# justinhj/minbpe-cc

Hardware: AMD Instinct MI355X
Metric: bpe_train_merges_per_sec (higher is better)
Workload: dtype u16; 1 GPU; BASELINE config 4: SplitMix64(seed 42) uniform-random bytes, 4294967296 bytes whole job, basic encoder (one chunk), vocab 32000, lexicographic tie-break; a step is ONE WHOLE TRAINING (pair-count scan, stream and table setup, every merge up to the vocabulary: 31744 merges); corpus_bytes=4294967296, vocab_size=32000

## Files before the change

### include/mbpe.h

```cpp
#ifndef MBPE_H
#define MBPE_H

#include <stdint.h>

#ifdef __cplusplus
extern "C" {
#endif

#define MBPE_API __attribute__((visibility("default")))

#define MBPE_MAX_VOCAB_BASIC   65534u
#define MBPE_MAX_VOCAB_ENDBIT  32766u
#define MBPE_MAX_VOCAB_CHUNKED 65518u
#define MBPE_MAX_VOCAB_WIDE    16777216u
#define MBPE_NO_BARRIER 0xFFFFFFFFu

typedef enum {
    MBPE_NEED_EXCHANGE =  1,
    MBPE_OK            =  0,
    MBPE_ERR_ARG       = -1,
    MBPE_ERR_NO_DEVICE = -2,
    MBPE_ERR_HIP       = -3,
    MBPE_ERR_VOCAB     = -4,
    MBPE_ERR_STATE     = -5,
// ... 76 lines not shown
MBPE_API int mbpe_train_sequences(mbpe_ctx *ctx, uint32_t n_sequences, uint32_t *merges_done_out);

MBPE_API int mbpe_train_result(mbpe_ctx *ctx, uint32_t *merges_out, int32_t *counts_out,
                               uint32_t cap_merges, uint32_t *n_merges_out);

MBPE_API int mbpe_train_lexical(mbpe_ctx *ctx, const uint8_t *text, uint64_t n_bytes,
                                const uint64_t *chunk_off, uint64_t n_chunks,
                                uint32_t vocab_size,
                                uint32_t *merges_out, int32_t *counts_out,
                                uint32_t *n_merges_out, mbpe_stats *stats_out);

MBPE_API int mbpe_train(mbpe_ctx *ctx, const uint8_t *text, uint64_t n_bytes,
                        const uint64_t *chunk_off, uint64_t n_chunks, uint32_t vocab_size,
                        int conflict_resolution,
                        uint32_t *merges_out, int32_t *counts_out,
                        uint32_t *n_merges_out, mbpe_stats *stats_out);

MBPE_API int mbpe_get_stats(mbpe_ctx *ctx, mbpe_stats *out);


MBPE_API int mbpe_get_stream(mbpe_ctx *ctx, uint32_t *tokens_out, uint8_t *chunk_end_out,
                             uint64_t cap, uint64_t *n_out);

MBPE_API int mbpe_stream_device(mbpe_ctx *ctx, const void **slots_out, uint64_t *n_slots_out,
                                uint32_t *slot_bits_out, uint32_t *end_bit_out, uint32_t *barrier_out);

MBPE_API int mbpe_table_device(mbpe_ctx *ctx, const void **cells_out, uint32_t *vshift_out);

MBPE_API int mbpe_get_pairs(mbpe_ctx *ctx, uint32_t *first_out, uint32_t *second_out,
                            int32_t *count_out, uint64_t cap, uint64_t *n_out);

MBPE_API int mbpe_compact(mbpe_ctx *ctx);

MBPE_API int mbpe_set_option(mbpe_ctx *ctx, const char *name, int64_t value);


MBPE_API int mbpe_encode_chunks(int device_id, const uint8_t *text, uint64_t n_bytes,
                                const uint64_t *chunk_off, uint64_t n_chunks,
                                const uint32_t *merges, uint32_t n_merges,
                                uint32_t *tokens_out, uint64_t cap, uint64_t *n_out,
                                uint32_t *n_passes_out);

MBPE_API int mbpe_encode_chunks_device(int device_id, const uint8_t *text, uint64_t n_bytes,
                                       const uint64_t *chunk_off, uint64_t n_chunks,
                                       const uint32_t *merges, uint32_t n_merges,
                                       uint32_t *tokens_dev_out, uint64_t cap, uint64_t *n_out,
                                       uint32_t *n_passes_out);

typedef struct mbpe_encoder mbpe_encoder;
MBPE_API int  mbpe_encoder_create(int device_id, const uint32_t *merges, uint32_t n_merges, mbpe_encoder **out);
MBPE_API void mbpe_encoder_destroy(mbpe_encoder *e);

MBPE_API int  mbpe_encoder_encode(mbpe_encoder *e, const uint8_t *text, uint64_t n_bytes, int text_on_device,
                                  const uint64_t *chunk_off, uint64_t n_chunks,
                                  void *tokens_out, uint64_t cap, uint32_t token_bits, int out_on_device,
                                  uint64_t *chunk_tok_off_out, uint64_t *n_out, uint32_t *n_passes_out);

MBPE_API int  mbpe_encoder_set_option(mbpe_encoder *e, const char *name, int64_t value);

MBPE_API int  mbpe_encoder_kernel_ms(const mbpe_encoder *e, float *ms_out);

MBPE_API int  mbpe_encoder_pass_tokens(const mbpe_encoder *e, uint64_t *tokens_out, uint32_t cap, uint32_t *n_out);

MBPE_API int  mbpe_encoder_alloc_count(const mbpe_encoder *e, uint64_t *n_out);


// ... 48 lines not shown
```

### minbpe-cc_amd/csrc/kernels.hip

```cpp
#include "mbpe_dev.h"
#include <hip/hip_ext.h>

#include <cstdlib>

namespace mbpe {

namespace {

constexpr int kWave = 64;
constexpr uint32_t kSent = 0x10000u;

__device__ __forceinline__ uint32_t lane_id() { return threadIdx.x & (kWave - 1); }
__device__ __forceinline__ uint32_t rfl(uint32_t v) { return __builtin_amdgcn_readfirstlane(v); }

typedef unsigned int u32x4 __attribute__((ext_vector_type(4)));

__device__ __forceinline__ uint32_t wave_from_next(uint32_t v, uint32_t edge) {
    return (uint32_t)__builtin_amdgcn_update_dpp((int)edge, (int)v, 0x130, 0xf, 0xf, false);
}
__device__ __forceinline__ uint32_t wave_from_prev(uint32_t v, uint32_t edge) {
    return (uint32_t)__builtin_amdgcn_update_dpp((int)edge, (int)v, 0x138, 0xf, 0xf, false);
}

#define MBPE_GLOBAL_AS __attribute__((address_space(1)))
// ... 583 lines not shown
            }
            const uint32_t issued = pc_generic_range(hist, bp, text, n, n_full, r_begin, v_end);
            __syncthreads();
            const PcCheck ck = pc_check(hist, issued, red);
            if (ck.sum != resid + ck.issued) {
#pragma unroll
                for (int k = 0; k < kPcWords / 4 / kPcThreads; ++k)
                    reinterpret_cast<uint4 *>(hist)[k * kPcThreads + threadIdx.x] =
                        resid ? my_snap[k * kPcThreads + threadIdx.x] : make_uint4(0, 0, 0, 0);
                __syncthreads();
                pc_slow_range(hist, bp, text, n, n_full, r_begin, v_end);
            }
        }
    }
    __syncthreads();
    PC_STAMP();
    pc_flush(hist, bp);
    const bool ends_here = n_full == 0 ? blockIdx.x == 0 : (v_begin < n_full && v_end == n_full);
    if (ends_here && threadIdx.x == 0) {
        uint64_t i = n_full * 16;
        if (i > 0 && !straddle_counted) --i;
        if (n_full * 16 == n) i = n;
        for (; i + 1 < n; ++i) atomicAdd(&bp[((uint32_t)text[i] << 8) | text[i + 1]], 1u);
    }
#ifdef MBPE_PC_STAMPS
    __builtin_amdgcn_s_waitcnt(0);
    __syncthreads();
    PC_STAMP();
    if (threadIdx.x == 0) for (; n_stamp < 16; ++n_stamp) stamps[n_stamp] = 0;
#endif
}


template <bool MASKED>
__global__ void k_widen(const uint8_t *__restrict__ text, uint64_t n, const uint8_t *__restrict__ endmask,
                        uint16_t *__restrict__ tok, uint64_t n_padded) {
    uint64_t vec = (uint64_t)blockIdx.x * blockDim.x + threadIdx.x;
    const uint64_t stride = (uint64_t)gridDim.x * blockDim.x;
    const uint64_t n_vec = n_padded / 16;
    for (; vec < n_vec; vec += stride) {
        const uint64_t byte0 = vec * 16;
        uint32_t w[4] = {0, 0, 0, 0};
        uint32_t ends = 0;
        if (byte0 + 16 <= n) {
            uint4 q = *reinterpret_cast<const uint4 *>(text + byte0);
            w[0] = q.x; w[1] = q.y; w[2] = q.z; w[3] = q.w;
        } else {
            for (uint64_t i = byte0; i < n; ++i)
                w[(i - byte0) >> 2] |= (uint32_t)text[i] << (8 * ((i - byte0) & 3));
        }
        if (MASKED && byte0 < n) ends = reinterpret_cast<const uint16_t *>(endmask)[vec];
        uint32_t o[8];
#pragma unroll
        for (int i = 0; i < 16; i += 2) {
            uint32_t t0 = (w[i >> 2] >> (8 * (i & 3))) & 0xFFu;
            uint32_t t1 = (w[(i + 1) >> 2] >> (8 * ((i + 1) & 3))) & 0xFFu;
            if (MASKED) {
                t0 |= ((ends >> i) & 1u) << 15;
                t1 |= ((ends >> (i + 1)) & 1u) << 15;
            }
            if (byte0 + i >= n) t0 = kHole;
            if (byte0 + i + 1 >= n) t1 = kHole;
            o[i >> 1] = t0 | (t1 << 16);
        }
        uint4 *dst = reinterpret_cast<uint4 *>(tok + byte0);
        dst[0] = make_uint4(o[0], o[1], o[2], o[3]);
        dst[1] = make_uint4(o[4], o[5], o[6], o[7]);
    }
}

__global__ void k_widen_barrier(const uint8_t *__restrict__ text, uint64_t n, const uint8_t *__restrict__ endmask,
                                uint16_t *__restrict__ tok, uint64_t n_slots) {
    uint64_t vec = (uint64_t)blockIdx.x * blockDim.x + threadIdx.x;
    const uint64_t stride = (uint64_t)gridDim.x * blockDim.x;
    const uint64_t n_vec = n_slots / 16;
    for (; vec < n_vec; vec += stride) {
        const uint64_t byte0 = vec * 8;
        uint32_t w[2] = {0, 0};
        uint32_t ends = 0;
        if (byte0 + 8 <= n) {
            const uint2 q = *reinterpret_cast<const uint2 *>(text + byte0);
            w[0] = q.x; w[1] = q.y;
        } else {
            for (uint64_t i = byte0; i < n; ++i) w[(i - byte0) >> 2] |= (uint32_t)text[i] << (8 * ((i - byte0) & 3));
        }
        if (byte0 < n) ends = endmask[vec];
        uint32_t o[8];
#pragma unroll
        for (int i = 0; i < 8; ++i) {
            uint32_t t = (w[i >> 2] >> (8 * (i & 3))) & 0xFFu;
            uint32_t e = ((ends >> i) & 1u) ? kBarrier : kHole;
            if (byte0 + i >= n) { t = kHole; e = kHole; }
            o[i] = t | (e << 16);
        }
        uint4 *dst = reinterpret_cast<uint4 *>(tok + vec * 16);
        dst[0] = make_uint4(o[0], o[1], o[2], o[3]);
        dst[1] = make_uint4(o[4], o[5], o[6], o[7]);
    }
}


template <int MODE>
// ... 225 lines not shown
    if (t == 0xFFFFFFFFu) return;
    const uint32_t nb = blockIdx.x, per = (nb + kRunThreads - 1) / kRunThreads;
    RunSeg acc = run_none();
    for (uint32_t i = threadIdx.x * per; i < nb && i < (threadIdx.x + 1) * per; ++i) acc = run_join(acc, run_unpack(part[i]));
    pre[threadIdx.x] = run_pack(acc);
    const uint64_t base = (uint64_t)blockIdx.x * kRunChunk;
    run_chunk_join(sin, n_tiles, base, segs, sh);
    if (threadIdx.x == 0) {
        RunSeg run = run_none();
        for (int i = 0; i < kRunThreads; ++i) run = run_join(run, run_unpack(pre[i]));
        for (int i = 0; i < kRunThreads; ++i) {
            const RunSeg mine = run_unpack(sh[i]);
            sh[i] = run_pack(run);
            run = run_join(run, mine);
        }
    }
    __syncthreads();
    RunSeg run = run_unpack(sh[threadIdx.x]);
    const unsigned long long edge = le ? ((unsigned long long)le->tail_run_hi << 32) | le->tail_run_lo : 0ull;
    const uint32_t edge_tok = le ? le->tail0 : kHole;
    for (int i = 0; i < kRunPerThread; ++i) {
        const uint32_t k = threadIdx.x * kRunPerThread + i;
        const bool reach = le && edge_tok != kHole && (run.empty || (run.full && run.token == edge_tok));
        const unsigned long long rb = run.len + (reach ? edge : 0ull);
        const RunSeg here = run_unpack(segs[k]);
        segs[k] = (rb & 1ull) | (rb >= 2 ? 2ull : 0ull);
        run = run_join(run, here);
    }
    __syncthreads();
    for (uint32_t i = threadIdx.x; i < kRunChunk; i += kRunThreads)
        if (base + i < n_tiles) run_in[base + i] = (uint32_t)segs[i];
}

__global__ __launch_bounds__(kMergeThreads) void k_summarize(const uint16_t *__restrict__ tok,
                                                             TileSum *__restrict__ sums, uint32_t n_tiles) {
    const uint32_t waves_per_block = kMergeThreads / kWave;
    const uint32_t n_waves = gridDim.x * waves_per_block;
    for (uint32_t tile = blockIdx.x * waves_per_block + threadIdx.x / kWave; tile < n_tiles; tile += n_waves) {
        const uint4 q = reinterpret_cast<const uint4 *>(tok)[(uint64_t)tile * kWave + lane_id()];
        uint32_t s[8];
        unpack8(q, s);
        uint4 sum;
        bool live = true;
#pragma unroll
        for (int j = 0; j < 8; ++j) live = live && s[j] != kHole;
        if (__ballot(!live) == 0ull) {
            const uint32_t lane = lane_id();
            const uint32_t t0 = rlane(s[7], kWave - 1);
            uint32_t last_diff = 0;
#pragma unroll
            for (int j = 0; j < 8; ++j) last_diff = s[j] != t0 ? (uint32_t)j + 1u : last_diff;
            const unsigned long long dm = __ballot(last_diff != 0u);
            uint32_t run = kTile;
            if (dm) {
                const uint32_t hl = 63u - (uint32_t)__builtin_clzll(dm);
                run = kTile - (hl * 8u + rlane(last_diff, hl));
            }
            sum = sum_to_u4(rlane(s[0], 0), rlane(s[1], 0), rlane(s[6], kWave - 1), t0, kTile, run);
            (void)lane;
        } else {
            sum = wave_summary(s);
        }
        if (lane_id() == 0) reinterpret_cast<uint4 *>(sums)[tile] = sum;
    }
}


constexpr int kArgmaxThreads = 256;

__global__ __launch_bounds__(kArgmaxThreads) void k_argmax(PairTable t, const DevCtl *ctl,
                                                           unsigned long long *best) {
    __shared__ unsigned long long wbest[kArgmaxThreads / kWave];
    const uint32_t n = table_size(t, ctl);
    unsigned long long b = 0;
    for (uint32_t i = blockIdx.x * blockDim.x + threadIdx.x; i < n; i += gridDim.x * blockDim.x) {
        const unsigned long long p = entry_packed(t, i);
        b = p > b ? p : b;
    }
    b = wave_max_u64(b);
    if (lane_id() == 0) wbest[threadIdx.x / kWave] = b;
    __syncthreads();
    if (threadIdx.x == 0) {
#pragma unroll
        for (int k = 1; k < kArgmaxThreads / kWave; ++k) b = wbest[k] > b ? wbest[k] : b;
        if (b) atomicMax(best, b);
    }
}

constexpr int kHierThreads = 256;
constexpr int kHierItems = kBlockSize / kHierThreads;

struct Top2 { unsigned long long v1, v2; uint32_t i1; };

__device__ __forceinline__ Top2 top2_merge(Top2 a, unsigned long long bv1, unsigned long long bv2, uint32_t bi1) {
    Top2 r;
    if (bv1 > a.v1) { r.v1 = bv1; r.i1 = bi1; r.v2 = a.v1 > bv2 ? a.v1 : bv2; }
// ... 1737 lines not shown
                }
            }
            outq = fused_tile_pf<MODE, DIAG, true, TT>(t0.q, s, h, old_x, old_y, old_z, lut, X0, tile, sout, hdr_adj, LR, dc,
                                                       dc_on, wave_rm, wrote_sum, lr_rsrc, adj_pitch, stage, chg, renamed, &ti,
                                                       need_rename, t_rsrc, use_t);
            if (TT && need_rename) {
                tt_rename<MODE>(s, h, ti, run_in[tile]);
                outq = fused_tile_pf<MODE, DIAG, true, TT>(t0.q, s, h, old_x, old_y, old_z, lut, X0, tile, sout, hdr_adj, LR,
                                                           dc, dc_on, wave_rm, wrote_sum, lr_rsrc, adj_pitch, stage, chg, true,
                                                           &ti, need_rename, t_rsrc, use_t);
            }
        }
        if (!wrote_sum && lane == 0) reinterpret_cast<uint4 *>(sout)[tile] = make_uint4(old_x, old_y, old_z, 0u);
        MBPE_GLOBAL_AS char *obase =
            (MBPE_GLOBAL_AS char *)uniform_ptr(reinterpret_cast<uintptr_t>(dst) + (uint64_t)tile * (kWave * 16u));
        u32x4 oq; oq.x = outq.x; oq.y = outq.y; oq.z = outq.z; oq.w = outq.w;
        __builtin_nontemporal_store(oq, (MBPE_GLOBAL_AS u32x4 *)(obase + lane * 16u));

        if (!v1) break;
        tile += n_waves;
#pragma unroll
        for (int d = 0; d + 1 < kDepth; ++d) ring[d] = ring[d + 1];
        ring[kDepth - 1] = t_new;
    }
    }
    if (dc_on) dc_flush(dc, LR);
    if (lane == 0 && wave_rm) atomicAdd(&ctl->rm, wave_rm);
    if (TT) {
        tt_flush(ti, hdr_m);
    }
}

__global__ __launch_bounds__(256) void k_pair_cells_fold(uint32_t *__restrict__ T, uint32_t *__restrict__ LR, const DevCtl *ctl) {
    __shared__ uint32_t rows[256];
    const uint32_t n = ctl->batch_n;
    if (n < ctl->cells_min || !ctl->cells_on) return;
    const uint32_t pitch = lr_pitch(256u + ctl->k_done);
    uint32_t hits = 0;
    const uint32_t t = threadIdx.x;
    for (uint32_t j = blockIdx.x; j < n; j += gridDim.x) {
        uint32_t *tj = T + (size_t)j * 65536u;
        rows[t] = 0;
        __syncthreads();
        uint32_t col = 0;
#pragma unroll 8
        for (uint32_t x = 0; x < 256u; ++x) {
            const uint32_t v = tj[x * 256u + t];
            if (__ballot(v != 0u) == 0ull) continue;
            if (v) tj[x * 256u + t] = 0;
            col += v;
            const uint32_t rs = wave_sum(v);
            if (lane_id() == 0 && rs) atomicAdd(&rows[x], rs);
        }
        __syncthreads();
        if (col) LR[lr_idx(pitch, t, j, 1u)] += col;
        if (rows[t]) LR[lr_idx(pitch, t, j, 0u)] += rows[t];
        hits += col;
        __syncthreads();
    }
    hits = wave_sum(hits);
    if (lane_id() == 0 && hits) atomicAdd(const_cast<uint32_t *>(&ctl->cell_hits), hits);
}


__global__ __launch_bounds__(kWave) void k_adj_sums(const uint32_t *__restrict__ hdr_adj, BatchState *bs, const DevCtl *ctl) {
    const uint32_t n = ctl->batch_n;
    if (n < 2) return;
    for (uint32_t j = blockIdx.x; j < n; j += gridDim.x) {
        uint32_t in = 0, out = 0;
        for (uint32_t p = threadIdx.x; p < n; p += kWave) { in += hdr_adj[p * ctl->adj_pitch + j]; out += hdr_adj[j * ctl->adj_pitch + p]; }
        in = wave_sum(in);
        out = wave_sum(out);
        if (threadIdx.x == 0) { bs->adj_in[j] = in; bs->adj_out[j] = out; }
    }
}

constexpr uint32_t kLrChunk = 4096;
__global__ __launch_bounds__(256) void k_delta_max(const uint32_t *__restrict__ LR, BatchState *bs, const DevCtl *ctl) {
    const uint32_t n_keys = ctl->batch_n;
    if (n_keys < 2) return;
    const uint32_t X = 256u + ctl->k_done;
    const uint32_t pitch = lr_pitch(X);
    const uint32_t chunks = (X + kLrChunk - 1u) / kLrChunk;
    const uint32_t n_items = 2u * n_keys * chunks;
    for (uint32_t item = blockIdx.x; item < n_items; item += gridDim.x) {
        const uint32_t row = item / chunks, x0 = (item - row * chunks) * kLrChunk;
        const uint32_t j = row >> 1, side = row & 1u, Xj = X + j;
// ... 771 lines not shown
        else if ((endbit) == kBarrier) { constexpr int M = 2; __VA_ARGS__; }               \
        else { constexpr int M = 0; __VA_ARGS__; }                                         \
    } while (0)

void launch_fill_u32(hipStream_t s, uint32_t *p, uint64_t n, uint32_t v) {
    if (!n) return;
    hipLaunchKernelGGL(k_fill_u32, dim3(blocks_for(n, 256, 4096)), dim3(256), 0, s, p, n, v);
}

void launch_fill_u16(hipStream_t s, uint16_t *p, uint64_t n, uint16_t v) {
    if (!n) return;
    hipLaunchKernelGGL(k_fill_u16, dim3(blocks_for(n, 256, 4096)), dim3(256), 0, s, p, n, v);
}

size_t pair_count_scratch_bytes(int n_workgroups) {
    const size_t wgs = (size_t)(n_workgroups < 1 ? 1 : n_workgroups);
    return wgs * kPcWords * 4 + wgs * 16 * 8;
}

void launch_pair_count_u8(hipStream_t s, const uint8_t *text, uint64_t n, const uint8_t *endmask,
                          uint32_t *bp, int n_workgroups, uint32_t *scratch, hipEvent_t start, hipEvent_t stop) {
    if (n < 2) return;
    uint64_t n_vec = n / 16;
    uint64_t max_wg = (n_vec + kPcThreads * kPcVpl - 1) / (kPcThreads * kPcVpl);
    if ((uint64_t)n_workgroups > max_wg) n_workgroups = (int)max_wg;
    if (n_workgroups < 1) n_workgroups = 1;
    if (endmask)
        hipExtLaunchKernelGGL(k_pair_count_u8<true>, dim3(n_workgroups), dim3(kPcThreads), 0, s, start, stop, 0, text, n, endmask, bp, scratch);
    else
        hipExtLaunchKernelGGL(k_pair_count_u8_fast, dim3(n_workgroups), dim3(kPcThreads), 0, s, start, stop, 0, text, n, bp, scratch);
}

void launch_widen(hipStream_t s, const uint8_t *text, uint64_t n, const uint8_t *endmask, uint16_t *tok,
                  uint64_t n_slots_padded) {
    if (!n_slots_padded) return;
    int blocks = blocks_for(n_slots_padded / 16, 256, 8192);
    if (endmask)
        hipLaunchKernelGGL(k_widen<true>, dim3(blocks), dim3(256), 0, s, text, n, endmask, tok, n_slots_padded);
    else
        hipLaunchKernelGGL(k_widen<false>, dim3(blocks), dim3(256), 0, s, text, n, endmask, tok, n_slots_padded);
}

void launch_widen_barrier(hipStream_t s, const uint8_t *text, uint64_t n, const uint8_t *endmask, uint16_t *tok,
                          uint64_t n_slots) {
    if (!n_slots) return;
    hipLaunchKernelGGL(k_widen_barrier, dim3(blocks_for(n_slots / 16, 256, 8192)), dim3(256), 0, s, text, n, endmask, tok,
                       n_slots);
}

void launch_summarize(hipStream_t s, const uint16_t *tok, TileSum *sums, uint32_t n_tiles, int n_cus) {
    if (!n_tiles) return;
    hipLaunchKernelGGL(k_summarize, dim3(tile_grid(n_tiles, n_cus)), dim3(kMergeThreads), 0, s, tok, sums, n_tiles);
}

void launch_table_init(hipStream_t s, const uint32_t *bp, PairTable t, DevCtl *ctl) {
    hipLaunchKernelGGL(k_table_init, dim3(65536 / 256), dim3(256), 0, s, bp, t, ctl);
}

void launch_table_rehash(hipStream_t s, PairTable t, DevCtl *ctl) {
    hipLaunchKernelGGL(k_table_rehash, dim3((t.ecap + 255) / 256), dim3(256), 0, s, t, ctl);
}

void launch_argmax(hipStream_t s, PairTable t, const DevCtl *ctl, unsigned long long *best, bool hierarchical) {
    if (hierarchical) {
        hipLaunchKernelGGL(k_argmax_hier, dim3(1), dim3(kHierThreads), 0, s, t, ctl, best);
        return;
    }
    int blocks = blocks_for(t.ecap, kArgmaxThreads * 4, 1024);
    hipLaunchKernelGGL(k_argmax, dim3(blocks), dim3(kArgmaxThreads), 0, s, t, ctl, best);
}

size_t first_state_bytes() { return sizeof(FirstState); }

// ... 292 lines not shown
```

### minbpe-cc_amd/csrc/mbpe_dev.h

```cpp
#ifndef MBPE_DEV_H
#define MBPE_DEV_H

#include <hip/hip_runtime.h>
#include <stdint.h>

namespace mbpe {

constexpr uint32_t kHole = 0xFFFFu;
constexpr uint32_t kEndBit = 0x8000u;
constexpr uint32_t kBarrier = 0xFFEEu;

constexpr int kTile = 512;
constexpr int kMergeThreads = 256;
#ifndef MBPE_LUT_THREADS
#define MBPE_LUT_THREADS 1024
#endif
constexpr int kLutThreads = MBPE_LUT_THREADS;
constexpr int kSlotsPerLane = 8;

struct __attribute__((aligned(16))) TileSum {
    uint16_t head0, head1;
    uint16_t tail1, tail0;
    uint16_t n_live;
    uint16_t tail_run;
// ... 121 lines not shown
    uint32_t skip_pos[kSkipMax];
    unsigned long long skip_packed[kSkipMax];
};

inline uint32_t batch_header_words(uint32_t adj_pitch) { return (uint32_t)kBatchMax + adj_pitch * adj_pitch; }
__host__ __device__ inline uint32_t lr_pitch(uint32_t ids) { return (ids + 63u) & ~63u; }
__host__ __device__ inline unsigned long long lr_words(uint32_t ids, uint32_t n_pairs) {
    return 2ull * (n_pairs ? n_pairs : 1u) * lr_pitch(ids);
}

constexpr uint32_t kErrTableFull   = 1u;
constexpr uint32_t kErrNegCount    = 2u;
constexpr uint32_t kErrMissingPair = 4u;
constexpr uint32_t kErrCountRange  = 8u;
constexpr uint32_t kErrHotSkipped  = 16u;

__host__ __device__ inline unsigned long long pack_best(int32_t count, uint32_t key) {
    return ((unsigned long long)(uint32_t)count << 32) | (uint32_t)(~key);
}

struct Launch {
    hipStream_t stream;
};

void launch_fill_u32(hipStream_t s, uint32_t *p, uint64_t n, uint32_t v);
void launch_fill_u16(hipStream_t s, uint16_t *p, uint64_t n, uint16_t v);

size_t pair_count_scratch_bytes(int n_workgroups);
void launch_pair_count_u8(hipStream_t s, const uint8_t *text, uint64_t n,
                          const uint8_t *endmask, uint32_t *bp, int n_workgroups, uint32_t *scratch,
                          hipEvent_t start = nullptr, hipEvent_t stop = nullptr);

void launch_widen(hipStream_t s, const uint8_t *text, uint64_t n, const uint8_t *endmask,
                  uint16_t *tok, uint64_t n_slots_padded);
void launch_widen_barrier(hipStream_t s, const uint8_t *text, uint64_t n, const uint8_t *endmask,
                          uint16_t *tok, uint64_t n_slots);

void launch_summarize(hipStream_t s, const uint16_t *tok, TileSum *sums, uint32_t n_tiles, int n_cus);

void launch_table_init(hipStream_t s, const uint32_t *bp, PairTable t, DevCtl *ctl);
void launch_table_rehash(hipStream_t s, PairTable t, DevCtl *ctl);

void launch_argmax(hipStream_t s, PairTable t, const DevCtl *ctl, unsigned long long *best, bool hierarchical);

size_t first_state_bytes();
void launch_first_init(hipStream_t s, void *fs);
void launch_first_tiebreak(hipStream_t s, PairTable t, const DevCtl *ctl, unsigned long long *best, void *fs,
                           const uint16_t *tok, const uint16_t *tok_other, const TileSum *sums, uint32_t n_tiles,
                           uint32_t endbit, int n_cus, int seq,
                           int phase = 0 ,
                           const RankEdge *right_edge = nullptr, uint32_t *xf = nullptr ,
                           int rank = 0, int n_ranks = 1);

void launch_merge(hipStream_t s, uint16_t *tok, uint16_t *tok_other, const TileSum *sums, TileSum *side,
                  uint32_t n_tiles, uint32_t *chg, const unsigned long long *best, uint32_t new_id,
                  uint32_t endbit, uint32_t *LR, DevCtl *ctl, uint32_t *m_adj ,
                  const RankEdge *left_edge, const RankEdge *right_edge, int n_cus, int seq,
                  unsigned long long *run_part ,
                  uint32_t *run_in ,
                  const BatchState *bs ,
                  int hot_possible = 1 ,
                  int only = -1 );
void launch_run_lengths(hipStream_t s, const TileSum *sums, uint32_t n_tiles, const unsigned long long *best, const DevCtl *ctl,
                        int seq, const BatchState *bs, unsigned long long *run_part, const RankEdge *left_edge, uint32_t *run_in);

void launch_apply(hipStream_t s, PairTable t, DevCtl *ctl, const unsigned long long *best,
                  uint32_t new_id, uint32_t *LR, const uint32_t *gm_gadj,
// ... 50 lines not shown
```

### minbpe-cc_amd/csrc/train.cpp

```cpp
#include "mbpe.h"
#include "mbpe_dev.h"
#include "wide.h"
#include "hip_host.h"

#include <dlfcn.h>
#include <rccl/rccl.h>

#include <algorithm>
#include <chrono>
#include <cstddef>
#include <cstdio>
#include <cstring>
#include <map>
#include <string>
#include <unordered_map>
#include <vector>

using namespace mbpe;

namespace {

#define HIPCHK(expr) MBPE_HIP_CHECK(expr, false)

uint64_t round_up(uint64_t v, uint64_t m) { return (v + m - 1) / m * m; }
// ... 776 lines not shown
        init.first_mode = c->opt_first ? 1u : 0u;
        init.adj_pitch = c->adj_pitch;
        init.cells_on = c->pair_cells ? 1u : 0u;
        init.cells_min = c->opt_pair_cells > 0 ? 2u : kCellsMinBatch;
        c->h_ctl = init;
        HIPCHK(hipMemcpyAsync(c->ctl, &c->h_ctl, sizeof(DevCtl), hipMemcpyHostToDevice, c->stream));
    }
    HIPCHK(hipMemsetAsync(c->best, 0, ((size_t)c->n_target + 2) * 8, c->stream));

    uint64_t want = 65536 + 2 * batch_headroom(c, (uint32_t)c->opt_batch);
    want = std::max<uint64_t>(want, n / 8);
    want = std::min<uint64_t>(want, table_cap_limit(c));
    int rc = use_dense(c) ? alloc_table_dense(c) : alloc_table(c, (uint32_t)want);
    if (rc != MBPE_OK) return rc;

    rc = ensure_pc_scratch(c);
    if (rc != MBPE_OK) return rc;
    pool_trim(c);
    HIPCHK(hipEventRecord(c->ev0, c->stream));
    if (n >= 2) launch_pair_count_u8(c->stream, c->d_text, n, c->d_endmask, c->xb0, c->n_cus, c->pc_scratch);
    c->cur = 0;
    if (c->barrier) {
        launch_widen_barrier(c->stream, c->d_text, n, c->d_endmask, c->tok[0], c->n_slots);
        launch_summarize(c->stream, c->tok[0], c->sums, c->n_tiles, c->n_cus);
        const double ms_compact = c->stats.ms_compact;
        rc = do_compact(c);
        if (rc != MBPE_OK) return rc;
        c->stats.n_compactions--;
        c->stats.ms_compact = ms_compact;
        tfree(c, c->tok[0]);
        pool_trim(c);
        HIPCHK(tmalloc(c, &c->tok[0], c->cap_slots * 2));
    } else {
        launch_widen(c->stream, c->d_text, n, c->d_endmask, c->tok[0], c->n_slots);
        launch_summarize(c->stream, c->tok[0], c->sums, c->n_tiles, c->n_cus);
    }
    if (is_multi(c)) {
        uint32_t *hdr = c->xb0 + 65536;
        launch_rank_edge(c->stream, c->sums, c->n_tiles, reinterpret_cast<RankEdge *>(hdr + 2) + c->rank, c->ctl, hdr);
        const uint64_t p = pairs_scanned(c);
        for (uint32_t i = 0; i < kPairCountWords; ++i) c->h_pcount[i] = (uint32_t)(p >> (16 * i)) & 0xFFFFu;
        HIPCHK(hipMemcpyAsync(hdr + c->hdr_words, c->h_pcount, sizeof(c->h_pcount), hipMemcpyHostToDevice, c->stream));
    }
    return MBPE_OK;
}

static void update_hot_possible(mbpe_ctx *c, unsigned long long top_count, uint64_t merges) {
    c->last_top = top_count;
    if (c->comm_external) { c->hot_possible = 1; return; }
    const unsigned long long live = c->h_ctl.n_live;
    const unsigned long long eaten = merges * top_count;
    c->hot_possible = !(live > eaten && top_count * 8192ull < (live - eaten) * (unsigned long long)std::max(1, c->n_ranks));
}

static inline bool first_sharded(const mbpe_ctx *c) { return c->opt_first && is_multi(c); }

static void begin_finish_a(mbpe_ctx *c) {
    const uint32_t endbit = endbit_of(c);
    if (is_multi(c)) {
        uint32_t *hdr = c->xb0 + 65536;
        launch_boundary_pairs(c->stream, c->xb0, hdr, c->n_ranks, endbit, hdr + c->hdr_words);
        launch_compose_edges(c->stream, hdr, c->rank, c->n_ranks, c->d_left, c->d_right);
        launch_pair_total(c->stream, c->xb0, hdr + c->hdr_words, 0, nullptr, c->ctl);
    } else {
        launch_pair_total(c->stream, c->xb0, nullptr, pairs_scanned(c), nullptr, c->ctl);
    }
    launch_table_init(c->stream, c->xb0, c->tab, c->ctl);
    launch_argmax(c->stream, c->tab, c->ctl, c->best, use_hier(c));
// ... 1024 lines not shown
            HIPCHK(hipMemcpy(rowbuf.data(), c->tab.cells + (size_t)tr * tpr * 1024, rowbuf.size() * 4,
                             hipMemcpyDeviceToHost));
            for (uint32_t fr = 0; fr < 32; ++fr)
                for (uint32_t tc = 0; tc < used_tiles; ++tc)
                    for (uint32_t sc = 0; sc < 32; ++sc) {
                        const uint32_t v = rowbuf[(size_t)tc * 1024 + fr * 32 + sc];
                        if (v & kPresent) recs.push_back({tr * 32 + fr, tc * 32 + sc, (int32_t)(v & ~kPresent)});
                    }
        }
        uint64_t o = recs.size();
        if (o > n) { mbpe_host::set_last_error("pair table holds more pairs than counted"); return MBPE_ERR_OVERFLOW; }
        for (uint64_t i = 0; i < o; ++i) {
            first_out[i] = recs[i].f;
            second_out[i] = recs[i].s;
            if (count_out) count_out[i] = recs[i].c;
        }
        if (o != n) { mbpe_host::set_last_error("pair table holds fewer pairs than counted"); return MBPE_ERR_OVERFLOW; }
        return MBPE_OK;
    }
    std::vector<uint32_t> keys(n);
    std::vector<int32_t> cnts(n);
    if (n) {
        HIPCHK(hipMemcpy(keys.data(), c->tab.ekey, n * 4, hipMemcpyDeviceToHost));
        HIPCHK(hipMemcpy(cnts.data(), c->tab.ecnt, n * 4, hipMemcpyDeviceToHost));
    }
    for (uint64_t i = 0; i < n; ++i) {
        first_out[i] = keys[i] >> 16;
        second_out[i] = keys[i] & 0xFFFFu;
        if (count_out) count_out[i] = cnts[i];
    }
    return MBPE_OK;
}

int mbpe_compact(mbpe_ctx *c) {
    if (!c) return MBPE_ERR_ARG;
    if (!c->begun) { mbpe_host::set_last_error("mbpe_compact before mbpe_train_begin"); return MBPE_ERR_STATE; }
    HIPCHK(hipSetDevice(c->device));
    if (c->wide_active) return MBPE_OK;
    int rc = sync_ctl(c);
    if (rc != MBPE_OK) return rc;
    return do_compact(c);
}


static int comm_allreduce(mbpe_ctx *c, uint32_t *buf, size_t count) {
    Rccl &r = rccl();
    if (!r.ok || !c->nccl_comm) { mbpe_host::set_last_error("RCCL communicator not initialised"); return MBPE_ERR_COMM; }
    int rc = r.AllReduce(buf, buf, count, (int)ncclUint32, (int)ncclSum, c->nccl_comm, c->stream);
    if (rc != 0) {
        mbpe_host::set_last_error(std::string("ncclAllReduce: ") + r.GetErrorString(rc));
        return MBPE_ERR_COMM;
    }
    return MBPE_OK;
}

int mbpe_comm_unique_id(uint8_t *id_out) {
    if (!id_out) return MBPE_ERR_ARG;
    Rccl &r = rccl();
    if (!r.ok) { mbpe_host::set_last_error(r.why); return MBPE_ERR_COMM; }
    static_assert(sizeof(ncclUniqueId) == MBPE_COMM_ID_BYTES, "unique id size");
    ncclUniqueId id;
    int rc = r.GetUniqueId(&id);
    if (rc != 0) { mbpe_host::set_last_error(std::string("ncclGetUniqueId: ") + r.GetErrorString(rc)); return MBPE_ERR_COMM; }
    memcpy(id_out, &id, sizeof(id));
    return MBPE_OK;
}
// ... 39 lines not shown
```

### minbpe-cc_amd/python/mbpe/__init__.py

```python
import ctypes
import os

import numpy as np

_PKG_DIR = os.path.dirname(os.path.dirname(os.path.dirname(os.path.abspath(__file__))))
LIB_PATH = os.environ.get("MBPE_LIB") or os.path.join(_PKG_DIR, "libmbpe.so")

OK = 0
NEED_EXCHANGE = 1
ERR_ARG, ERR_NO_DEVICE, ERR_HIP, ERR_VOCAB, ERR_STATE = -1, -2, -3, -4, -5
ERR_OOM, ERR_REGEX, ERR_SPLIT_GAP, ERR_COMM, ERR_OVERFLOW, ERR_IO = -6, -7, -8, -9, -10, -11
COMM_ID_BYTES = 128

EXPORTS = [
    "mbpe_last_error", "mbpe_version", "mbpe_create", "mbpe_destroy", "mbpe_load_corpus",
    "mbpe_pair_count_u8", "mbpe_train_begin", "mbpe_train_steps", "mbpe_train_sequences", "mbpe_train_result",
    "mbpe_train_lexical", "mbpe_train", "mbpe_get_stats", "mbpe_get_stream", "mbpe_stream_device", "mbpe_table_device", "mbpe_get_pairs", "mbpe_compact",
    "mbpe_set_option", "mbpe_comm_unique_id", "mbpe_comm_init", "mbpe_comm_init_external",
    "mbpe_comm_exchange_buffer", "mbpe_comm_exchange_done", "mbpe_presplit",
    "mbpe_split_count", "mbpe_split_offsets", "mbpe_split_has_gaps", "mbpe_split_starts", "mbpe_split_ends",
    "mbpe_split_free", "mbpe_load_corpus_ranges", "mbpe_split_pattern", "mbpe_encode_chunks",
    "mbpe_encode_chunks_device", "mbpe_decoder_create", "mbpe_decoder_destroy", "mbpe_decode_tokens",
    "mbpe_decode_slots", "mbpe_decoder_kernel_ms", "mbpe_decode_stream", "mbpe_encoder_create",
    "mbpe_encoder_destroy", "mbpe_encoder_encode", "mbpe_encoder_set_option", "mbpe_encoder_kernel_ms",
    "mbpe_encoder_alloc_count", "mbpe_encoder_pass_tokens",
]
TOK_EXPORTS = [
    "mbpe_tok_create", "mbpe_tok_destroy", "mbpe_tok_set_special_tokens", "mbpe_tok_train", "mbpe_tok_set_merges",
    "mbpe_tok_get_merges", "mbpe_tok_save", "mbpe_tok_load", "mbpe_tok_encode", "mbpe_tok_encode_device",
    "mbpe_tok_decode", "mbpe_tok_decode_device", "mbpe_tok_encode_batch_device",
]


class Stats(ctypes.Structure):
    _fields_ = [
        ("n_bytes", ctypes.c_uint64), ("n_chunks", ctypes.c_uint64), ("n_slots", ctypes.c_uint64),
        ("n_live", ctypes.c_uint64), ("n_merges", ctypes.c_uint32), ("n_compactions", ctypes.c_uint32),
        ("n_pairs", ctypes.c_uint64), ("ms_pair_count", ctypes.c_float), ("ms_begin", ctypes.c_float),
        ("ms_steps", ctypes.c_float), ("pair_count_launches", ctypes.c_uint32), ("merge_launches", ctypes.c_uint32),
        ("ms_merge_kernel", ctypes.c_float), ("n_batches", ctypes.c_uint32),
        ("n_fused", ctypes.c_uint32), ("n_fused_dropped", ctypes.c_uint32), ("cut_conflict", ctypes.c_uint32),
        ("cut_bucket", ctypes.c_uint32), ("cut_single", ctypes.c_uint32), ("cut_full", ctypes.c_uint32),
        ("n_validation_drops", ctypes.c_uint32), ("ms_grow_table", ctypes.c_float), ("ms_compact", ctypes.c_float),
        ("n_table_grows", ctypes.c_uint32), ("n_sel_fallback", ctypes.c_uint32),
        ("fused_launches", ctypes.c_uint32), ("ms_fused_kernel", ctypes.c_float), ("fused_slots", ctypes.c_uint64),
        ("n_sel_retry", ctypes.c_uint32), ("adapt_limit", ctypes.c_uint32), ("n_sel_blocks", ctypes.c_uint64), ("size_hist", ctypes.c_uint32 * 8),
        ("n_skipped", ctypes.c_uint32), ("n_skip_cut", ctypes.c_uint32),
        ("exchange_words", ctypes.c_uint64), ("exchanges", ctypes.c_uint32), ("pad_", ctypes.c_uint32),
        ("fused_live_tokens", ctypes.c_uint64), ("ms_pair_count_kernel", ctypes.c_float), ("pad2_", ctypes.c_uint32),
    ]
# ... 12 lines not shown


_lib = None


def lib():
    global _lib
    if _lib is not None:
        return _lib
    if not os.path.exists(LIB_PATH):
        raise ImportError("libmbpe.so is not built (%s); run __graft_entry__.build()" % LIB_PATH)
    L = ctypes.CDLL(LIB_PATH)
    vp, u64, u32, i32, i64 = ctypes.c_void_p, ctypes.c_uint64, ctypes.c_uint32, ctypes.c_int, ctypes.c_int64
    L.mbpe_last_error.restype = ctypes.c_char_p
    L.mbpe_version.restype = ctypes.c_char_p
    L.mbpe_create.argtypes = [i32, ctypes.POINTER(vp)]
    L.mbpe_destroy.argtypes = [vp]
    L.mbpe_destroy.restype = None
    L.mbpe_load_corpus.argtypes = [vp, vp, u64, vp, u64, i32]
    L.mbpe_pair_count_u8.argtypes = [vp, vp]
    L.mbpe_train_begin.argtypes = [vp, u32]
    L.mbpe_train_steps.argtypes = [vp, u32, vp]
    L.mbpe_train_sequences.argtypes = [vp, u32, vp]
    L.mbpe_train_result.argtypes = [vp, vp, vp, u32, vp]
    L.mbpe_train_lexical.argtypes = [vp, vp, u64, vp, u64, u32, vp, vp, vp, vp]
    L.mbpe_train.argtypes = [vp, vp, u64, vp, u64, u32, i32, vp, vp, vp, vp]
    L.mbpe_get_stats.argtypes = [vp, vp]
    L.mbpe_get_stream.argtypes = [vp, vp, vp, u64, vp]
    L.mbpe_stream_device.argtypes = [vp, ctypes.POINTER(vp), ctypes.POINTER(u64), ctypes.POINTER(u32), ctypes.POINTER(u32),
                                     ctypes.POINTER(u32)]
    L.mbpe_table_device.argtypes = [vp, ctypes.POINTER(vp), ctypes.POINTER(u32)]
    L.mbpe_get_pairs.argtypes = [vp, vp, vp, vp, u64, vp]
    L.mbpe_compact.argtypes = [vp]
    L.mbpe_set_option.argtypes = [vp, ctypes.c_char_p, i64]
    L.mbpe_comm_unique_id.argtypes = [vp]
    L.mbpe_comm_init.argtypes = [vp, vp, i32, i32]
    L.mbpe_comm_init_external.argtypes = [vp, i32, i32]
    L.mbpe_comm_exchange_buffer.argtypes = [vp, ctypes.POINTER(vp), ctypes.POINTER(u64)]
    L.mbpe_comm_exchange_done.argtypes = [vp]
    L.mbpe_presplit.argtypes = [ctypes.c_char_p, vp, u64, ctypes.POINTER(vp)]
    L.mbpe_split_count.argtypes = [vp]
    L.mbpe_split_count.restype = u64
    L.mbpe_split_offsets.argtypes = [vp]
    L.mbpe_split_offsets.restype = ctypes.POINTER(ctypes.c_uint64)
    L.mbpe_split_has_gaps.argtypes = [vp]
    L.mbpe_split_starts.argtypes = [vp]
    L.mbpe_split_starts.restype = ctypes.POINTER(ctypes.c_uint64)
    L.mbpe_split_ends.argtypes = [vp]
    L.mbpe_split_ends.restype = ctypes.POINTER(ctypes.c_uint64)
    L.mbpe_load_corpus_ranges.argtypes = [vp, vp, u64, vp, vp, u64, i32]
    L.mbpe_split_free.argtypes = [vp]
    L.mbpe_split_free.restype = None
    L.mbpe_split_pattern.argtypes = [ctypes.c_char_p]
    L.mbpe_split_pattern.restype = ctypes.c_char_p
    L.mbpe_encode_chunks.argtypes = [i32, vp, u64, vp, u64, vp, u32, vp, u64, vp, vp]
    L.mbpe_encode_chunks_device.argtypes = [i32, vp, u64, vp, u64, vp, u32, vp, u64, vp, vp]
    L.mbpe_encoder_create.argtypes = [i32, vp, u32, ctypes.POINTER(vp)]
    L.mbpe_encoder_destroy.argtypes = [vp]
    L.mbpe_encoder_destroy.restype = None
    L.mbpe_encoder_encode.argtypes = [vp, vp, u64, i32, vp, u64, vp, u64, u32, i32, vp, vp, vp]
    L.mbpe_encoder_set_option.argtypes = [vp, ctypes.c_char_p, i64]
    L.mbpe_encoder_kernel_ms.argtypes = [vp, vp]
    L.mbpe_encoder_alloc_count.argtypes = [vp, vp]
    L.mbpe_encoder_pass_tokens.argtypes = [vp, vp, u32, vp]
    L.mbpe_tok_encode_batch_device.argtypes = [vp, vp, vp, u64, i32, i32, vp, u64, vp, vp]
    L.mbpe_decoder_create.argtypes = [i32, vp, u32, vp, vp, vp, u32, ctypes.POINTER(vp)]
# ... 373 lines not shown
    def decode_stream(self):
        n = ctypes.c_uint64()
        _check(lib().mbpe_decode_stream(self._h, None, 0, 0, ctypes.byref(n)))
        out = np.zeros(max(n.value, 1), dtype=np.uint8)
        _check(lib().mbpe_decode_stream(self._h, out.ctypes.data, n.value, 0, ctypes.byref(n)))
        return out[:n.value].tobytes()

    def decode_stream_device(self, out_ptr, cap):
        n = ctypes.c_uint64()
        _check(lib().mbpe_decode_stream(self._h, ctypes.c_void_p(out_ptr) if out_ptr else None, cap, 1, ctypes.byref(n)))
        return n.value

    def table_device(self):
        p, v = ctypes.c_void_p(), ctypes.c_uint32()
        _check(lib().mbpe_table_device(self._h, ctypes.byref(p), ctypes.byref(v)))
        return p.value, v.value

    def pairs(self):
        n = ctypes.c_uint64()
        _check(lib().mbpe_get_pairs(self._h, None, None, None, 0, ctypes.byref(n)))
        a = np.zeros(max(n.value, 1), dtype=np.uint32)
        b = np.zeros(max(n.value, 1), dtype=np.uint32)
        c = np.zeros(max(n.value, 1), dtype=np.int32)
        _check(lib().mbpe_get_pairs(self._h, a.ctypes.data, b.ctypes.data, c.ctypes.data, n.value, ctypes.byref(n)))
        return a[:n.value], b[:n.value], c[:n.value]

    def pairs_dict(self):
        a, b, c = self.pairs()
        return {(int(x), int(y)): int(z) for x, y, z in zip(a, b, c)}

    def compact(self):
        _check(lib().mbpe_compact(self._h))

    def comm_init(self, uid, rank, n_ranks):
        buf = (ctypes.c_uint8 * COMM_ID_BYTES).from_buffer_copy(bytes(uid))
        _check(lib().mbpe_comm_init(self._h, buf, rank, n_ranks))


def comm_unique_id():
    buf = (ctypes.c_uint8 * COMM_ID_BYTES)()
    _check(lib().mbpe_comm_unique_id(buf))
    return bytes(buf)


class Tokenizer:

    FIRST, LEXICAL = 0, 1

    def __init__(self, pattern=""):
        self._h = ctypes.c_void_p()
        _check(lib().mbpe_tok_create(pattern.encode("utf-8"), ctypes.byref(self._h)))

    def close(self):
        if self._h:
            lib().mbpe_tok_destroy(self._h)
            self._h = ctypes.c_void_p()

    def __del__(self):
        try:
            self.close()
        except Exception:
            pass

    def set_special_tokens_from_file(self, text):
        b = text if isinstance(text, bytes) else text.encode("utf-8")
        _check(lib().mbpe_tok_set_special_tokens(self._h, b, len(b)))
# ... 63 lines not shown
```

Measured before the change: 81170 merges/s.

## Fuse tile summarization into widen kernel and restructure pair-cell fold

The widen kernel is rewritten to run per wave over groups of tiles and to compute each tile's summary as it writes the widened u16 tokens. This removes the separate summarize pass that re-read the whole token stream. The pair-cell fold kernel now uses vectorised nontemporal 128-bit loads several rows deep and per-wave column partials in shared memory, replacing the scalar row loop and its shared atomics. A debug API for reading tile sums is added for verification.

```diff
diff --git a/include/mbpe.h b/include/mbpe.h
--- a/include/mbpe.h
+++ b/include/mbpe.h
@@ -132,6 +132,8 @@
 
 MBPE_API int mbpe_compact(mbpe_ctx *ctx);
 
+MBPE_API int mbpe_debug_tile_sums(mbpe_ctx *ctx, void *sums_out, uint64_t cap_tiles, uint64_t *n_tiles_out);
+
 MBPE_API int mbpe_set_option(mbpe_ctx *ctx, const char *name, int64_t value);
 
 
diff --git a/minbpe-cc_amd/csrc/kernels.hip b/minbpe-cc_amd/csrc/kernels.hip
--- a/minbpe-cc_amd/csrc/kernels.hip
+++ b/minbpe-cc_amd/csrc/kernels.hip
@@ -639,42 +639,6 @@
 }
 
 
-template <bool MASKED>
-__global__ void k_widen(const uint8_t *__restrict__ text, uint64_t n, const uint8_t *__restrict__ endmask,
-                        uint16_t *__restrict__ tok, uint64_t n_padded) {
-    uint64_t vec = (uint64_t)blockIdx.x * blockDim.x + threadIdx.x;
-    const uint64_t stride = (uint64_t)gridDim.x * blockDim.x;
-    const uint64_t n_vec = n_padded / 16;
-    for (; vec < n_vec; vec += stride) {
-        const uint64_t byte0 = vec * 16;
-        uint32_t w[4] = {0, 0, 0, 0};
-        uint32_t ends = 0;
-        if (byte0 + 16 <= n) {
-            uint4 q = *reinterpret_cast<const uint4 *>(text + byte0);
-            w[0] = q.x; w[1] = q.y; w[2] = q.z; w[3] = q.w;
-        } else {
-            for (uint64_t i = byte0; i < n; ++i)
-                w[(i - byte0) >> 2] |= (uint32_t)text[i] << (8 * ((i - byte0) & 3));
-        }
-        if (MASKED && byte0 < n) ends = reinterpret_cast<const uint16_t *>(endmask)[vec];
-        uint32_t o[8];
-#pragma unroll
-        for (int i = 0; i < 16; i += 2) {
-            uint32_t t0 = (w[i >> 2] >> (8 * (i & 3))) & 0xFFu;
-            uint32_t t1 = (w[(i + 1) >> 2] >> (8 * ((i + 1) & 3))) & 0xFFu;
-            if (MASKED) {
-                t0 |= ((ends >> i) & 1u) << 15;
-                t1 |= ((ends >> (i + 1)) & 1u) << 15;
-            }
-            if (byte0 + i >= n) t0 = kHole;
-            if (byte0 + i + 1 >= n) t1 = kHole;
-            o[i >> 1] = t0 | (t1 << 16);
-        }
-        uint4 *dst = reinterpret_cast<uint4 *>(tok + byte0);
-        dst[0] = make_uint4(o[0], o[1], o[2], o[3]);
-        dst[1] = make_uint4(o[4], o[5], o[6], o[7]);
-    }
-}
 
 __global__ void k_widen_barrier(const uint8_t *__restrict__ text, uint64_t n, const uint8_t *__restrict__ endmask,
                                 uint16_t *__restrict__ tok, uint64_t n_slots) {
@@ -966,6 +930,20 @@
         if (base + i < n_tiles) run_in[base + i] = (uint32_t)segs[i];
 }
 
+__device__ __forceinline__ uint4 full_tile_summary(const uint32_t s[8]) {
+    const uint32_t t0 = rlane(s[7], kWave - 1);
+    uint32_t last_diff = 0;
+#pragma unroll
+    for (int j = 0; j < 8; ++j) last_diff = s[j] != t0 ? (uint32_t)j + 1u : last_diff;
+    const unsigned long long dm = __ballot(last_diff != 0u);
+    uint32_t run = kTile;
+    if (dm) {
+        const uint32_t hl = 63u - (uint32_t)__builtin_clzll(dm);
+        run = kTile - (hl * 8u + rlane(last_diff, hl));
+    }
+    return sum_to_u4(rlane(s[0], 0), rlane(s[1], 0), rlane(s[6], kWave - 1), t0, kTile, run);
+}
+
 __global__ __launch_bounds__(kMergeThreads) void k_summarize(const uint16_t *__restrict__ tok,
                                                              TileSum *__restrict__ sums, uint32_t n_tiles) {
     const uint32_t waves_per_block = kMergeThreads / kWave;
@@ -974,28 +952,58 @@
         const uint4 q = reinterpret_cast<const uint4 *>(tok)[(uint64_t)tile * kWave + lane_id()];
         uint32_t s[8];
         unpack8(q, s);
-        uint4 sum;
         bool live = true;
 #pragma unroll
         for (int j = 0; j < 8; ++j) live = live && s[j] != kHole;
-        if (__ballot(!live) == 0ull) {
-            const uint32_t lane = lane_id();
-            const uint32_t t0 = rlane(s[7], kWave - 1);
-            uint32_t last_diff = 0;
-#pragma unroll
-            for (int j = 0; j < 8; ++j) last_diff = s[j] != t0 ? (uint32_t)j + 1u : last_diff;
-            const unsigned long long dm = __ballot(last_diff != 0u);
-            uint32_t run = kTile;
-            if (dm) {
-                const uint32_t hl = 63u - (uint32_t)__builtin_clzll(dm);
-                run = kTile - (hl * 8u + rlane(last_diff, hl));
-            }
-            sum = sum_to_u4(rlane(s[0], 0), rlane(s[1], 0), rlane(s[6], kWave - 1), t0, kTile, run);
-            (void)lane;
-        } else {
-            sum = wave_summary(s);
-        }
+        const uint4 sum = __ballot(!live) == 0ull ? full_tile_summary(s) : wave_summary(s);
         if (lane_id() == 0) reinterpret_cast<uint4 *>(sums)[tile] = sum;
+    }
+}
+
+
+constexpr uint32_t kWidenGroup = 4;
+template <bool MASKED>
+__global__ __launch_bounds__(kMergeThreads) void k_widen(const uint8_t *__restrict__ text, uint64_t n,
+                                                         const uint8_t *__restrict__ endmask, uint16_t *__restrict__ tok,
+                                                         TileSum *__restrict__ sums, uint32_t n_tiles) {
+    const uint32_t waves_per_block = kMergeThreads / kWave;
+    const uint32_t n_waves = gridDim.x * waves_per_block;
+    const uint32_t lane = lane_id();
+    const uint32_t n_groups = (n_tiles + kWidenGroup - 1u) / kWidenGroup;
+    for (uint32_t g = blockIdx.x * waves_per_block + threadIdx.x / kWave; g < n_groups; g += n_waves) {
+        uint2 w[kWidenGroup];
+        uint32_t ends[kWidenGroup];
+#pragma unroll
+        for (uint32_t k = 0; k < kWidenGroup; ++k) {
+            const uint64_t byte0 = ((uint64_t)(g * kWidenGroup + k) * kWave + lane) * 8u;
+            w[k] = make_uint2(0u, 0u);
+            ends[k] = 0;
+            if (byte0 + 8 <= n) {
+                w[k] = *reinterpret_cast<const uint2 *>(text + byte0);
+            } else {
+                for (uint64_t i = byte0; i < n; ++i) {
+                    const uint32_t b = (uint32_t)text[i] << (8 * ((i - byte0) & 3));
+                    if (i - byte0 < 4) w[k].x |= b; else w[k].y |= b;
+                }
+            }
+            if (MASKED && byte0 < n) ends[k] = endmask[byte0 >> 3];
+        }
+#pragma unroll
+        for (uint32_t k = 0; k < kWidenGroup; ++k) {
+            const uint32_t tile = g * kWidenGroup + k;
+            if (tile >= n_tiles) break;
+            const uint64_t byte0 = ((uint64_t)tile * kWave + lane) * 8u;
+            uint32_t s[8];
+#pragma unroll
+            for (int i = 0; i < 8; ++i) {
+                uint32_t t = ((i < 4 ? w[k].x : w[k].y) >> (8 * (i & 3))) & 0xFFu;
+                if (MASKED) t |= ((ends[k] >> i) & 1u) << 15;
+                s[i] = byte0 + i < n ? t : kHole;
+            }
+            reinterpret_cast<uint4 *>(tok)[(uint64_t)tile * kWave + lane] = pack8(s);
+            const uint4 sum = ((uint64_t)tile + 1u) * kTile <= n ? full_tile_summary(s) : wave_summary(s);
+            if (lane == 0) reinterpret_cast<uint4 *>(sums)[tile] = sum;
+        }
     }
 }
 
@@ -2799,27 +2807,43 @@
 }
 
 __global__ __launch_bounds__(256) void k_pair_cells_fold(uint32_t *__restrict__ T, uint32_t *__restrict__ LR, const DevCtl *ctl) {
+    constexpr uint32_t kFoldWaves = 256 / kWave, kFoldDepth = 8;
     __shared__ uint32_t rows[256];
+    __shared__ uint32_t cols[kFoldWaves][256];
     const uint32_t n = ctl->batch_n;
     if (n < ctl->cells_min || !ctl->cells_on) return;
     const uint32_t pitch = lr_pitch(256u + ctl->k_done);
     uint32_t hits = 0;
-    const uint32_t t = threadIdx.x;
+    const uint32_t t = threadIdx.x, lane = lane_id(), wave = t / kWave;
     for (uint32_t j = blockIdx.x; j < n; j += gridDim.x) {
-        uint32_t *tj = T + (size_t)j * 65536u;
-        rows[t] = 0;
+        MBPE_GLOBAL_AS u32x4 *tj = (MBPE_GLOBAL_AS u32x4 *)(T + (size_t)j * 65536u);
+        uint32_t c0 = 0, c1 = 0, c2 = 0, c3 = 0;
+        for (uint32_t x0 = wave; x0 < 256u; x0 += kFoldWaves * kFoldDepth) {
+            u32x4 v[kFoldDepth];
+#pragma unroll
+            for (uint32_t k = 0; k < kFoldDepth; ++k)
+                v[k] = __builtin_nontemporal_load(tj + (x0 + k * kFoldWaves) * 64u + lane);
+#pragma unroll
+            for (uint32_t k = 0; k < kFoldDepth; ++k) {
+                const uint32_t x = x0 + k * kFoldWaves;
+                uint32_t rs = 0;
+                if (__ballot((v[k].x | v[k].y | v[k].z | v[k].w) != 0u) != 0ull) {
+                    if ((v[k].x | v[k].y | v[k].z | v[k].w) != 0u) {
+                        u32x4 z; z.x = 0; z.y = 0; z.z = 0; z.w = 0;
+                        tj[x * 64u + lane] = z;
+                    }
+                    c0 += v[k].x; c1 += v[k].y; c2 += v[k].z; c3 += v[k].w;
+                    rs = wave_sum(v[k].x + v[k].y + v[k].z + v[k].w);
+                }
+                if (lane == 0) rows[x] = rs;
+            }
+        }
+        cols[wave][lane * 4u + 0u] = c0; cols[wave][lane * 4u + 1u] = c1;
+        cols[wave][lane * 4u + 2u] = c2; cols[wave][lane * 4u + 3u] = c3;
         __syncthreads();
         uint32_t col = 0;
-#pragma unroll 8
-        for (uint32_t x = 0; x < 256u; ++x) {
-            const uint32_t v = tj[x * 256u + t];
-            if (__ballot(v != 0u) == 0ull) continue;
-            if (v) tj[x * 256u + t] = 0;
-            col += v;
-            const uint32_t rs = wave_sum(v);
-            if (lane_id() == 0 && rs) atomicAdd(&rows[x], rs);
-        }
-        __syncthreads();
+#pragma unroll
+        for (uint32_t w = 0; w < kFoldWaves; ++w) col += cols[w][t];
         if (col) LR[lr_idx(pitch, t, j, 1u)] += col;
         if (rows[t]) LR[lr_idx(pitch, t, j, 0u)] += rows[t];
         hits += col;
@@ -3657,13 +3681,13 @@
 }
 
 void launch_widen(hipStream_t s, const uint8_t *text, uint64_t n, const uint8_t *endmask, uint16_t *tok,
-                  uint64_t n_slots_padded) {
-    if (!n_slots_padded) return;
-    int blocks = blocks_for(n_slots_padded / 16, 256, 8192);
+                  TileSum *sums, uint32_t n_tiles, int n_cus) {
+    if (!n_tiles) return;
+    const dim3 grid(tile_grid((n_tiles + kWidenGroup - 1u) / kWidenGroup, n_cus)), block(kMergeThreads);
     if (endmask)
-        hipLaunchKernelGGL(k_widen<true>, dim3(blocks), dim3(256), 0, s, text, n, endmask, tok, n_slots_padded);
+        hipLaunchKernelGGL(k_widen<true>, grid, block, 0, s, text, n, endmask, tok, sums, n_tiles);
     else
-        hipLaunchKernelGGL(k_widen<false>, dim3(blocks), dim3(256), 0, s, text, n, endmask, tok, n_slots_padded);
+        hipLaunchKernelGGL(k_widen<false>, grid, block, 0, s, text, n, endmask, tok, sums, n_tiles);
 }
 
 void launch_widen_barrier(hipStream_t s, const uint8_t *text, uint64_t n, const uint8_t *endmask, uint16_t *tok,
diff --git a/minbpe-cc_amd/csrc/mbpe_dev.h b/minbpe-cc_amd/csrc/mbpe_dev.h
--- a/minbpe-cc_amd/csrc/mbpe_dev.h
+++ b/minbpe-cc_amd/csrc/mbpe_dev.h
@@ -177,7 +177,7 @@
                           hipEvent_t start = nullptr, hipEvent_t stop = nullptr);
 
 void launch_widen(hipStream_t s, const uint8_t *text, uint64_t n, const uint8_t *endmask,
-                  uint16_t *tok, uint64_t n_slots_padded);
+                  uint16_t *tok, TileSum *sums, uint32_t n_tiles, int n_cus);
 void launch_widen_barrier(hipStream_t s, const uint8_t *text, uint64_t n, const uint8_t *endmask,
                           uint16_t *tok, uint64_t n_slots);
 
diff --git a/minbpe-cc_amd/csrc/train.cpp b/minbpe-cc_amd/csrc/train.cpp
--- a/minbpe-cc_amd/csrc/train.cpp
+++ b/minbpe-cc_amd/csrc/train.cpp
@@ -832,8 +832,7 @@
         pool_trim(c);
         HIPCHK(tmalloc(c, &c->tok[0], c->cap_slots * 2));
     } else {
-        launch_widen(c->stream, c->d_text, n, c->d_endmask, c->tok[0], c->n_slots);
-        launch_summarize(c->stream, c->tok[0], c->sums, c->n_tiles, c->n_cus);
+        launch_widen(c->stream, c->d_text, n, c->d_endmask, c->tok[0], c->sums, c->n_tiles, c->n_cus);
     }
     if (is_multi(c)) {
         uint32_t *hdr = c->xb0 + 65536;
@@ -1924,6 +1923,19 @@
     return MBPE_OK;
 }
 
+int mbpe_debug_tile_sums(mbpe_ctx *c, void *sums_out, uint64_t cap_tiles, uint64_t *n_tiles_out) {
+    if (!c || !n_tiles_out) return MBPE_ERR_ARG;
+    if (!c->begun) { mbpe_host::set_last_error("mbpe_debug_tile_sums before mbpe_train_begin"); return MBPE_ERR_STATE; }
+    HIPCHK(hipSetDevice(c->device));
+    HIPCHK(hipStreamSynchronize(c->stream));
+    const uint64_t n = c->wide_active ? 0 : c->n_tiles;
+    *n_tiles_out = n;
+    if (!sums_out) return MBPE_OK;
+    if (cap_tiles < n) { mbpe_host::set_last_error("sums_out too small"); return MBPE_ERR_ARG; }
+    if (n) HIPCHK(hipMemcpy(sums_out, c->sums, n * sizeof(TileSum), hipMemcpyDeviceToHost));
+    return MBPE_OK;
+}
+
 int mbpe_compact(mbpe_ctx *c) {
     if (!c) return MBPE_ERR_ARG;
     if (!c->begun) { mbpe_host::set_last_error("mbpe_compact before mbpe_train_begin"); return MBPE_ERR_STATE; }
diff --git a/minbpe-cc_amd/python/mbpe/__init__.py b/minbpe-cc_amd/python/mbpe/__init__.py
--- a/minbpe-cc_amd/python/mbpe/__init__.py
+++ b/minbpe-cc_amd/python/mbpe/__init__.py
@@ -16,6 +16,7 @@
     "mbpe_last_error", "mbpe_version", "mbpe_create", "mbpe_destroy", "mbpe_load_corpus",
     "mbpe_pair_count_u8", "mbpe_train_begin", "mbpe_train_steps", "mbpe_train_sequences", "mbpe_train_result",
     "mbpe_train_lexical", "mbpe_train", "mbpe_get_stats", "mbpe_get_stream", "mbpe_stream_device", "mbpe_table_device", "mbpe_get_pairs", "mbpe_compact",
+    "mbpe_debug_tile_sums",
     "mbpe_set_option", "mbpe_comm_unique_id", "mbpe_comm_init", "mbpe_comm_init_external",
     "mbpe_comm_exchange_buffer", "mbpe_comm_exchange_done", "mbpe_presplit",
     "mbpe_split_count", "mbpe_split_offsets", "mbpe_split_has_gaps", "mbpe_split_starts", "mbpe_split_ends",
@@ -94,6 +95,7 @@
     L.mbpe_table_device.argtypes = [vp, ctypes.POINTER(vp), ctypes.POINTER(u32)]
     L.mbpe_get_pairs.argtypes = [vp, vp, vp, vp, u64, vp]
     L.mbpe_compact.argtypes = [vp]
+    L.mbpe_debug_tile_sums.argtypes = [vp, vp, u64, ctypes.POINTER(u64)]
     L.mbpe_set_option.argtypes = [vp, ctypes.c_char_p, i64]
     L.mbpe_comm_unique_id.argtypes = [vp]
     L.mbpe_comm_init.argtypes = [vp, vp, i32, i32]
@@ -533,6 +535,13 @@
     def compact(self):
         _check(lib().mbpe_compact(self._h))
 
+    def tile_sums(self):
+        n = ctypes.c_uint64()
+        _check(lib().mbpe_debug_tile_sums(self._h, None, 0, ctypes.byref(n)))
+        out = np.zeros((max(n.value, 1), 8), dtype=np.uint16)
+        _check(lib().mbpe_debug_tile_sums(self._h, out.ctypes.data, n.value, ctypes.byref(n)))
+        return out[:n.value]
+
     def comm_init(self, uid, rank, n_ranks):
         buf = (ctypes.c_uint8 * COMM_ID_BYTES).from_buffer_copy(bytes(uid))
         _check(lib().mbpe_comm_init(self._h, buf, rank, n_ranks))
```

Result: no change. 81640 merges/s, median of 6 (+0.6%).
